# duckietown/gym-duckietown

Measured on NVIDIA H100. Metric: env-steps/sec (obs+reward+done) at N envs, 1/2/4/8 H100 vs CPU ref, higher is better.
Workload: dtype f64 logic / f32 raster / u8 obs

## Files before the change

gym-duckietown_b200/csrc/dts_maps.cu:

```cuda
#include <cstdarg>
#include <cstdio>
#include <cstring>
#include <type_traits>
#include <utility>
#include <vector>

#include "dts_kernels.h"

namespace dts {

struct MapSlot {
  DMap rec{};
  std::vector<void*> allocs;
  uint64_t hash = 0;
};

struct MapSlots {
  int n_envs;
  DMap* table = nullptr;
  std::vector<MapSlot> slots;
  std::vector<MapCounts> counts;
};

MapSlots* maps_create(const dts_config& cfg) {
  const size_t bytes = sizeof(DMap) * cfg.max_maps;
  void* t = nullptr;
  if (cudaMalloc(&t, bytes) != cudaSuccess) return nullptr;
  cudaMemset(t, 0, bytes);
  return new MapSlots{cfg.num_envs, static_cast<DMap*>(t), std::vector<MapSlot>(cfg.max_maps),
                      std::vector<MapCounts>(cfg.max_maps)};
}

void maps_destroy(MapSlots* m) {
  if (!m) return;
  for (const MapSlot& s : m->slots)
    for (void* p : s.allocs) cudaFree(p);
  cudaFree(m->table);
  delete m;
}

const DMap* maps_table(const MapSlots& m) { return m.table; }

const DMap* maps_get(const MapSlots& m, int slot) {
  return slot >= 0 && slot < (int)m.slots.size() && m.slots[slot].rec.valid ? &m.slots[slot].rec : nullptr;
}

const std::vector<MapCounts>& maps_counts(const MapSlots& m) { return m.counts; }

int maps_slot_count(const MapSlots& m) { return (int)m.slots.size(); }

uint64_t maps_hash(const MapSlots& m, int slot) { return maps_get(m, slot) ? m.slots[slot].hash : 0; }

namespace {
struct Hasher {
  uint64_t h = 0xcbf29ce484222325ull;
  void bytes(const void* p, size_t n) {
    const uint8_t* b = static_cast<const uint8_t*>(p);
    size_t i = 0;
    for (; i + 8 <= n; i += 8) {
      uint64_t w;
      memcpy(&w, b + i, 8);
      h = (h ^ w) * 0x100000001b3ull;
    }
    for (; i < n; i++) h = (h ^ b[i]) * 0x100000001b3ull;
  }
  template <typename T> void arr(const T* p, size_t count) {
    const uint64_t c = p ? count : 0;
    bytes(&c, sizeof c);
    if (p && count) bytes(p, count * sizeof(T));
  }
  template <typename T> void val(const T& v) { bytes(&v, sizeof v); }
  uint64_t done() const {
    uint64_t z = h;
    z = (z ^ (z >> 30)) * 0xbf58476d1ce4e5b9ull;
    z = (z ^ (z >> 27)) * 0x94d049bb133111ebull;
    z ^= z >> 31;
    return z ? z : 1;
  }
};
}

static uint64_t blob_hash(const dts_map_blob& b) {
  Hasher H;
  const size_t T = (size_t)b.grid_w * b.grid_h;
  H.val(b.tile_size); H.val(b.grid_w); H.val(b.grid_h);
  H.arr(b.tile_kind, T); H.arr(b.tile_angle, T); H.arr(b.tile_drivable, T); H.arr(b.tile_tex, T);
  H.arr(b.tile_curve_off, T); H.arr(b.tile_curve_cnt, T);
  H.arr(b.curves, (size_t)b.n_curves * 12);
  H.arr(b.coll_corners, (size_t)b.n_coll * 8); H.arr(b.coll_norms, (size_t)b.n_coll * 4);
  H.arr(b.coll_centers, (size_t)b.n_coll * 3); H.arr(b.coll_radii, (size_t)b.n_coll);
  H.val(b.n_objects);
  for (int o = 0; o < b.n_objects; o++) { dts_object s = b.objects[o]; s.reserved = 0; H.val(s); }
  H.val(b.n_meshes);
  for (int i = 0; i < b.n_meshes; i++) { dts_mesh s = b.meshes[i]; s.reserved = 0; H.val(s); }
  H.arr(b.tri_pos, (size_t)b.n_tris * 9); H.arr(b.tri_nrm, (size_t)b.n_tris * 9); H.arr(b.tri_uv, (size_t)b.n_tris * 6);
  H.arr(b.tri_col, (size_t)b.n_tris * 9); H.arr(b.tri_tex, (size_t)b.n_tris);
  H.val(b.n_textures);
  for (int t = 0; t < b.n_textures; t++) {
    const dts_texture& s = b.textures[t];
    H.val(s.width); H.val(s.height);
    H.arr(s.rgba, (size_t)s.width * s.height * 4);
  }
  H.arr(b.tex_segment, b.tex_segment ? (size_t)b.n_textures : 0);
  if (b.tex_class) {
    size_t texels = 0;
    for (int t = 0; t < b.n_textures; t++) texels += (size_t)b.textures[t].width * b.textures[t].height;
    H.arr(b.tex_class, texels);
  }
  H.val(b.start_tile[0]); H.val(b.start_tile[1]); H.val(b.has_start_pose);
  for (int k = 0; k < 3; k++) H.val(b.start_pose[k]);
  H.val(b.agent_mesh);
  H.val(b.n_dyn);
  for (int s = 0; s < b.n_dyn; s++) { dts_dyn_object q = b.dyn[s]; q.reserved = 0; H.val(q); }
  return H.done();
}

static std::string format(const char* fmt, ...) {
  char buf[512];
  va_list ap;
  va_start(ap, fmt);
  vsnprintf(buf, sizeof buf, fmt, ap);
  va_end(ap);
  return buf;
}

static size_t pool_bytes(const dts_texture& s) { return ((size_t)s.width * s.height * 4 + 255) & ~size_t(255); }

static std::string validate(const dts_map_blob* b, int slot, int n_slots) {
  if (!b || slot < 0 || slot >= n_slots) return format("bad map_id %d", slot);
  if (b->n_objects > DTS_MAX_OBJECTS) return format("map has %d objects, limit %d", b->n_objects, DTS_MAX_OBJECTS);
  if (b->grid_w <= 0 || b->grid_h <= 0 || !(b->tile_size > 0)) return "invalid tile grid";
  if (b->n_dyn < 0 || b->n_dyn > DTS_MAX_DYN) return format("map has %d dynamic obstacles, limit %d", b->n_dyn, DTS_MAX_DYN);
  for (int o = 0; o < b->n_objects; o++) {
    const dts_object& s = b->objects[o];
    if (s.mesh_id < 0 || s.mesh_id >= b->n_meshes) return format("object %d: bad mesh_id", o);
    if (s.alt_tex_to >= b->n_textures || s.alt_tex_from >= b->n_textures) return format("object %d: alt texture out of range", o);
    if (s.dyn_slot >= b->n_dyn) return format("object %d: dyn_slot %d out of range", o, s.dyn_slot);
  }
  for (int i = 0; i < b->n_meshes; i++) {
    const dts_mesh& me = b->meshes[i];
    if (me.tri_offset < 0 || me.tri_count < 0 || (int64_t)me.tri_offset + me.tri_count > b->n_tris)
      return format("mesh %d: triangles %d .. %d past n_tris %d", i, me.tri_offset, me.tri_offset + me.tri_count, b->n_tris);
  }
  size_t pool = 0;
  for (int t = 0; t < b->n_textures; t++) {
    const dts_texture& s = b->textures[t];
    if (s.width <= 0 || s.height <= 0 || (s.width & (s.width - 1)) || (s.height & (s.height - 1)))
      return format("texture %d: %dx%d is not a power of two", t, s.width, s.height);
    if (s.width > (1 << 15) || s.height > (1 << 15)) return format("texture %d: %dx%d too large", t, s.width, s.height);
    pool += pool_bytes(s);
  }
  if (pool >= (size_t(1) << 32)) return "textures exceed 4 GB";
  for (int s = 0; s < b->n_dyn; s++) {
    const dts_dyn_object& q = b->dyn[s];
    if (q.kind != DTS_DYN_DUCKIE && q.kind != DTS_DYN_DUCKIEBOT && q.kind != DTS_DYN_TRAFFICLIGHT) return format("dyn %d: bad kind %d", s, q.kind);
    if (q.object_index < 0 || q.object_index >= b->n_objects || b->objects[q.object_index].dyn_slot != s)
      return format("dyn %d: object_index %d does not point back to this slot", s, q.object_index);
  }
  return "";
}

static DObject mesh_object(const dts_map_blob& b, int mesh_id, float& top) {
  const dts_mesh& me = b.meshes[mesh_id];
  DObject d{};
  d.mesh_id = mesh_id; d.tri_offset = me.tri_offset; d.tri_count = me.tri_count;
  d.seg_tex = (me.seg_flat_tex >= 0 && me.seg_flat_tex < b.n_textures) ? me.seg_flat_tex : -1;
  float lo[3] = {1e30f, 1e30f, 1e30f}, hi[3] = {-1e30f, -1e30f, -1e30f};
  for (int t = 0; t < me.tri_count * 3; t++)
    for (int k = 0; k < 3; k++) {
      const float v = b.tri_pos[((size_t)me.tri_offset * 3 + t) * 3 + k];
      lo[k] = v < lo[k] ? v : lo[k];
      hi[k] = v > hi[k] ? v : hi[k];
    }
  top = hi[0] > hi[1] ? hi[0] : hi[1];
  top = top > hi[2] ? top : hi[2];
  float r2 = 0.f;
  for (int k = 0; k < 3; k++) { d.centre[k] = 0.5f * (lo[k] + hi[k]); const float h = 0.5f * (hi[k] - lo[k]); r2 += h * h; }
  d.bound_rad = sqrtf(r2);
  return d;
}

template <typename T>
static std::string upload(T*& dst, const std::remove_const_t<T>* src, size_t count, std::vector<void*>& owned) {
  const size_t bytes = (count ? count : 1) * sizeof(T);
  void* d = nullptr;
  cudaError_t e = cudaMalloc(&d, bytes + 16);
  if (e != cudaSuccess) return format("cudaMalloc(%zu B) failed: %s", bytes, cudaGetErrorString(e));
  owned.push_back(d);
  cudaMemset(d, 0, bytes + 16);
  if (count && src && (e = cudaMemcpy(d, src, count * sizeof(T), cudaMemcpyHostToDevice)) != cudaSuccess)
    return format("cudaMemcpy H2D failed: %s", cudaGetErrorString(e));
  dst = static_cast<T*>(d);
  return "";
}

std::string maps_upload(MapSlots& ms, int slot, const dts_map_blob* blob) {
  std::string err = validate(blob, slot, (int)ms.slots.size());
  if (!err.empty()) return err;
  const dts_map_blob& b = *blob;
  DMap m{};
  const size_t T = (size_t)b.grid_w * b.grid_h;
  m.tile_size = b.tile_size; m.grid_w = b.grid_w; m.grid_h = b.grid_h; m.n_tiles = (int)T;
  m.n_coll = b.n_coll;
  std::vector<int32_t> drv;
  for (int j = 0; j < b.grid_h; j++)
    for (int i = 0; i < b.grid_w; i++)
      if (b.tile_kind[j * b.grid_w + i] >= 0 && b.tile_drivable[j * b.grid_w + i]) { drv.push_back(i); drv.push_back(j); }
  m.start_i = b.start_tile[0]; m.start_j = b.start_tile[1];
  if (m.start_i < 0 || m.start_j < 0 || m.start_i >= b.grid_w || m.start_j >= b.grid_h) { m.start_i = -1; m.start_j = -1; }
  m.has_start_pose = b.has_start_pose != 0;
  for (int k = 0; k < 3; k++) m.start_pose[k] = b.start_pose[k];
  m.n_drivable = (int)drv.size() / 2;
  MapCounts counts{m.n_tiles, b.n_objects, 0};
  std::vector<DObject> objs(b.n_objects);
  for (int o = 0; o < b.n_objects; o++) {
    const dts_object& s = b.objects[o];
    float top;
    DObject& d = objs[o] = mesh_object(b, s.mesh_id, top);
    d.tri_base = (int32_t)counts.n_tris;
    for (int k = 0; k < 3; k++) { d.pos[k] = (float)s.pos[k]; d.dpos[k] = s.pos[k]; }
    d.dyn_slot = s.dyn_slot;
    d.alt_from = s.alt_tex_from; d.alt_to = s.alt_tex_to;
    d.scale = s.scale; d.y_rot_deg = s.y_rot_deg; d.optional = s.optional;
    d.spawn_rad = top * 0.5f * s.scale + 0.25f;
    counts.n_tris += d.tri_count;
  }
  m.n_objects = b.n_objects;
  m.n_tris = b.n_tris;
  if (b.agent_mesh >= 0 && b.agent_mesh < b.n_meshes) {
    float top;
    m.agent = mesh_object(b, b.agent_mesh, top);
    m.agent.scale = 1.0f; m.agent.dyn_slot = -1; m.agent.alt_from = m.agent.alt_to = -1;
  }
  m.agent.tri_base = (int32_t)counts.n_tris;
  counts.n_tris += m.agent.tri_count;
  std::vector<DTexture> tex(b.n_textures);
  std::vector<size_t> off(b.n_textures);
  size_t pool_size = 0;
  for (int t = 0; t < b.n_textures; t++) {
    off[t] = pool_size;
    pool_size += pool_bytes(b.textures[t]);
  }
  const size_t class_off = pool_size ? pool_size : 256;
  std::vector<uint8_t> pool(class_off + class_off / 4, 0);
  size_t class_src = 0;
  for (int t = 0; t < b.n_textures; t++) {
    const dts_texture& s = b.textures[t];
    memcpy(pool.data() + off[t], s.rgba, (size_t)s.width * s.height * 4);
    if (b.tex_class) memcpy(pool.data() + class_off + off[t] / 4, b.tex_class + class_src, (size_t)s.width * s.height);
    class_src += (size_t)s.width * s.height;
    int lw = 0, lh = 0;
    while ((1 << lw) < s.width) lw++;
    while ((1 << lh) < s.height) lh++;
    tex[t].w = s.width; tex[t].h = s.height;
    tex[t].info = (uint32_t)(off[t] >> 8) | ((uint32_t)lw << 24) | ((uint32_t)lh << 28);
    tex[t].pad = 0;
  }
  m.n_textures = b.n_textures;
  m.tex_class_off = (uint32_t)class_off;
  std::vector<int16_t> seg(b.n_textures > 0 ? b.n_textures : 1);
  for (int t = 0; t < b.n_textures; t++) {
    const int v = b.tex_segment ? b.tex_segment[t] : -1;
    seg[t] = (int16_t)((v >= 0 && v < b.n_textures) ? v : t);
  }
  m.n_dyn = b.n_dyn;
  const size_t N = ms.n_envs, D = b.n_dyn;
  std::vector<DDyn> par(D);
  std::vector<double> st((size_t)DTS_DYN_FIELDS * D * N);
  for (size_t s = 0; s < D; s++) {
    const dts_dyn_object& q = b.dyn[s];
    DDyn& p = par[s];
    p.kind = q.kind; p.object_index = q.object_index; p.pos_y = q.pos[1];
    for (int k = 0; k < 4; k++) p.norms[k] = q.norms[k / 2][k % 2];
    p.safety_radius = q.safety_radius; p.walk_distance = q.walk_distance; p.wiggle = q.wiggle; p.angle0 = q.angle;
    p.follow_dist = q.follow_dist; p.velocity = q.velocity; p.gain = q.gain; p.trim = q.trim; p.radius = q.radius;
    p.k = q.k; p.limit = q.limit; p.wheel_dist = q.wheel_dist; p.robot_width = q.robot_width; p.robot_length = q.robot_length;
    double f[DTS_DYN_FIELDS] = {};
    f[DTS_DYN_PX] = q.pos[0]; f[DTS_DYN_PZ] = q.pos[2]; f[DTS_DYN_ANGLE] = q.angle;
    f[DTS_DYN_YROT] = q.angle * (180.0 / 3.14159265358979323846);
    for (int k = 0; k < 4; k++) { f[DTS_DYN_CORNERS + 2 * k] = q.corners[k][0]; f[DTS_DYN_CORNERS + 2 * k + 1] = q.corners[k][1]; }
    f[DTS_DYN_START_X] = q.pos[0]; f[DTS_DYN_START_Z] = q.pos[2];
    f[DTS_DYN_WAIT] = q.wait_time; f[DTS_DYN_VEL] = q.vel; f[DTS_DYN_TIME] = 0.0; f[DTS_DYN_ACTIVE] = 0.0;
    p.freq = q.freq; p.tl_first = -1; p.pad = 0;
    if (q.kind == DTS_DYN_TRAFFICLIGHT) f[DTS_DYN_PATTERN] = q.pattern ? 1.0 : 0.0;
    for (int k = 0; k < DTS_DYN_FIELDS; k++)
      for (size_t e = 0; e < N; e++) st[((size_t)k * D + s) * N + e] = f[k];
  }
  int tl_first = -1, tl_last = -1;
  for (size_t s = 0; s < D; s++)
    if (par[s].kind == DTS_DYN_TRAFFICLIGHT) { if (tl_first < 0) tl_first = (int)s; tl_last = (int)s; }
  for (size_t s = 0; s < D; s++) par[s].tl_first = tl_first;
  if (tl_first >= 0)
    for (size_t e = 0; e < N; e++) st[((size_t)DTS_DYN_SHOWN * D + tl_first) * N + e] = b.dyn[tl_last].pattern ? 1.0 : 0.0;
  std::vector<double> init((size_t)DTS_DYN_FIELDS * D);
  for (int k = 0; k < DTS_DYN_FIELDS; k++)
    for (size_t s = 0; s < D; s++) init[(size_t)k * D + s] = N ? st[((size_t)k * D + s) * N] : 0.0;
  MapSlot fresh;
  auto put = [&](auto*& dst, const auto* src, size_t count) { if (err.empty()) err = upload(dst, src, count, fresh.allocs); };
  put(m.tile_kind, b.tile_kind, T);
  put(m.tile_angle, b.tile_angle, T);
  put(m.tile_drivable, b.tile_drivable, T);
  put(m.tile_tex, b.tile_tex, T);
  put(m.tile_curve_off, b.tile_curve_off, T);
  put(m.tile_curve_cnt, b.tile_curve_cnt, T);
  put(m.curves, b.curves, (size_t)b.n_curves * 12);
  put(m.coll_corners, b.coll_corners, (size_t)b.n_coll * 8);
  put(m.coll_norms, b.coll_norms, (size_t)b.n_coll * 4);
  put(m.coll_centers, b.coll_centers, (size_t)b.n_coll * 3);
  put(m.coll_radii, b.coll_radii, (size_t)b.n_coll);
  put(m.drivable_ij, drv.data(), drv.size());
  put(m.objects, objs.data(), objs.size());
  put(m.tri_pos, b.tri_pos, (size_t)b.n_tris * 9);
  put(m.tri_nrm, b.tri_nrm, (size_t)b.n_tris * 9);
  put(m.tri_uv, b.tri_uv, (size_t)b.n_tris * 6);
  put(m.tri_col, b.tri_col, (size_t)b.n_tris * 9);
  put(m.tri_tex, b.tri_tex, (size_t)b.n_tris);
  put(m.tex_pool, pool.data(), pool.size());
  for (int t = 0; t < b.n_textures && err.empty(); t++) tex[t].rgba = m.tex_pool + off[t];
  put(m.textures, tex.data(), tex.size());
  put(m.tex_segment, seg.data(), seg.size());
  put(m.dyn, par.data(), par.size());
  put(m.dyn_state, st.data(), st.size());
  put(m.dyn_init, init.data(), init.size());
  m.valid = 1;
  if (err.empty()) {
    cudaError_t e = cudaDeviceSynchronize();
    if (e == cudaSuccess) e = cudaMemcpy(ms.table + slot, &m, sizeof(DMap), cudaMemcpyHostToDevice);
    if (e != cudaSuccess) err = format("map table update failed: %s", cudaGetErrorString(e));
  }
  if (err.empty()) {
    fresh.rec = m;
    fresh.hash = blob_hash(b);
    std::swap(ms.slots[slot], fresh);
    ms.counts[slot] = counts;
  }
  for (void* p : fresh.allocs) cudaFree(p);
  return err;
}

}
```

gym-duckietown_b200/csrc/dts_render.cu:

```cuda
#include <algorithm>
#include <cstddef>
#include <cstdlib>
#include <iterator>
#include <type_traits>
#include <utility>
#include <vector>

#include "dts_camera.cuh"
#include "dts_kernels.h"

namespace dts {

struct RemapTab {
  const int32_t* src_xy;
  const short4* cbox;
  const short4* fbox;
  const int32_t* cell_start;
  const uint16_t* cell_bins;
  const int32_t* home_start;
  const int4* home_ent;
  int ext_x, ext_y;
  const uint16_t* table_of_env;
};
constexpr int kRemapNone = 0, kRemapTable = 1, kRemapPool = 2;
// ... 202 lines not shown
  const Vtx* vs[3] = {&a, &b, &c};
  int X[3], Y[3];
  float zw[3], q[3];
  const float Wf = (float)ec.W, Hf = (float)ec.H;
#pragma unroll
  for (int k = 0; k < 3; k++) {
    const float iw = 1.0f / vs[k]->cw;
    const float nx = vs[k]->cx * iw, ny = vs[k]->cy * iw, nz = vs[k]->cz * iw;
    const float sx = (nx * 0.5f + 0.5f) * Wf;
    const float sy = (0.5f - ny * 0.5f) * Hf;
    X[k] = (int)rintf(sx * 64.0f);
    Y[k] = (int)rintf(sy * 64.0f);
    zw[k] = nz * 0.5f + 0.5f;
    q[k] = iw;
  }
  const long long area2 = (long long)(X[1] - X[0]) * (Y[2] - Y[0]) - (long long)(X[2] - X[0]) * (Y[1] - Y[0]);
  if (area2 == 0) return false;
  const int i1 = area2 < 0 ? 2 : 1, i2 = area2 < 0 ? 1 : 2;
  const int x0 = X[0], y0 = Y[0], x1 = X[i1], y1 = Y[i1], x2 = X[i2], y2 = Y[i2];
  int minx = min(x0, min(x1, x2)), maxx = max(x0, max(x1, x2));
  int miny = min(y0, min(y1, y2)), maxy = max(y0, max(y1, y2));
  int qx[4] = {x0, x1, x2, 0}, qy[4] = {y0, y1, y2, 0};
  if (d) {
    const float iw = 1.0f / d->cw;
    const float sx = ((d->cx * iw) * 0.5f + 0.5f) * Wf, sy = (0.5f - (d->cy * iw) * 0.5f) * Hf;
    const int X3 = (int)rintf(sx * 64.0f), Y3 = (int)rintf(sy * 64.0f);
    if (area2 > 0) { qx[1] = X[1]; qy[1] = Y[1]; qx[2] = X[2]; qy[2] = Y[2]; qx[3] = X3; qy[3] = Y3; }
    else { qx[1] = X3; qy[1] = Y3; qx[2] = X[2]; qy[2] = Y[2]; qx[3] = X[1]; qy[3] = Y[1]; }
#pragma unroll
    for (int k = 0; k < 4; k++) {
      const int k1 = (k + 1) & 3, k2 = (k + 2) & 3;
      const long long cr = (long long)(qx[k1] - qx[k]) * (qy[k2] - qy[k1]) - (long long)(qx[k2] - qx[k1]) * (qy[k1] - qy[k]);
      if (cr <= 0) return false;
    }
    minx = min(minx, X3); maxx = max(maxx, X3); miny = min(miny, Y3); maxy = max(maxy, Y3);
  }
  const int px0 = max(minx >> 6, 0), px1 = min(maxx >> 6, ec.W - 1);
  const int py0 = max(miny >> 6, 0), py1 = min(maxy >> 6, ec.H - 1);
  if (px0 > px1 || py0 > py1) return true;
  if (!d && (maxx >> 6) - (minx >> 6) < 3 && (maxy >> 6) - (miny >> 6) < 3) {
    const int ex[3] = {x1 - x0, x2 - x1, x0 - x2}, ey[3] = {y1 - y0, y2 - y1, y0 - y2};
    const int ax[3] = {0, x1 - x0, x2 - x0}, ay[3] = {0, y1 - y0, y2 - y0};
    int e00[3];
#pragma unroll
    for (int k = 0; k < 3; k++) {
      const int bias = (ey[k] > 0 || (ey[k] == 0 && ex[k] < 0)) ? 0 : 1;
      e00[k] = ex[k] * (py0 * kSub - y0 - ay[k]) - ey[k] * (px0 * kSub - x0 - ax[k]) - bias;
    }
    bool any = false;
    for (int py = 0; py <= py1 - py0; py++)
      for (int px = 0; px <= px1 - px0; px++) {
#pragma unroll
        for (int s = 0; s < 4; s++) {
          const int sx = px * kSub + sample_x(s), sy = py * kSub + sample_y(s);
          const int e0 = e00[0] + ex[0] * sy - ey[0] * sx, e1 = e00[1] + ex[1] * sy - ey[1] * sx, e2 = e00[2] + ex[2] * sy - ey[2] * sx;
          any |= (e0 | e1 | e2) >= 0;
        }
      }
    if (!any) return true;
  }
  PrimRec r;
  r.X0 = x0; r.Y0 = y0; r.X1 = x1; r.Y1 = y1; r.X2 = x2; r.Y2 = y2; r.X3 = x0; r.Y3 = y0;
  const float dx1 = (float)(x1 - x0) * 0.015625f, dy1 = (float)(y1 - y0) * 0.015625f;
  const float dx2 = (float)(x2 - x0) * 0.015625f, dy2 = (float)(y2 - y0) * 0.015625f;
  const float areaf = dx1 * dy2 - dx2 * dy1;
  const float ia = 1.0f / areaf;
  const Vtx* p0 = vs[0]; const Vtx* p1 = vs[i1]; const Vtx* p2 = vs[i2];
  const float q0 = q[0], q1 = q[i1], q2 = q[i2];
  const float v0[7] = {zw[0], q0, p0->u * q0, p0->v * q0, p0->r * q0, p0->g * q0, p0->b * q0};
  const float v1[7] = {zw[i1], q1, p1->u * q1, p1->v * q1, p1->r * q1, p1->g * q1, p1->b * q1};
  const float v2[7] = {zw[i2], q2, p2->u * q2, p2->v * q2, p2->r * q2, p2->g * q2, p2->b * q2};
  float f0[7], fx[7], fy[7];
#pragma unroll
  for (int at = 0; at < 7; at++) {
    const float d1 = v1[at] - v0[at], d2 = v2[at] - v0[at];
    f0[at] = v0[at];
    fx[at] = (d1 * dy2 - d2 * dy1) * ia;
    fy[at] = (d2 * dx1 - d1 * dx2) * ia;
  }
  r.z0 = f0[0]; r.zx = fx[0]; r.zy = fy[0];
  r.q0 = f0[1]; r.qx = fx[1]; r.qy = fy[1];
  r.u0 = f0[2]; r.ux = fx[2]; r.uy = fy[2];
  r.v0 = f0[3]; r.vx = fx[3]; r.vy = fy[3];
  r.r0 = f0[4]; r.rx = fx[4]; r.ry = fy[4];
  r.g0 = f0[5]; r.gx = fx[5]; r.gy = fy[5];
  r.b0 = f0[6]; r.bx = fx[6]; r.by = fy[6];
  r.id = id;
  r.ltq = (lat + 1) | ((tex + 1) << 16);
  r.tex = tex >= 0 ? ec.textures[tex].info : 0u;
  if (d) {
    r.ltq |= 1 << 24;
    r.X1 = qx[1]; r.Y1 = qy[1]; r.X2 = qx[2]; r.Y2 = qy[2]; r.X3 = qx[3]; r.Y3 = qy[3];
  }
  const unsigned act = __activemask();
  const int lane = threadIdx.x & 31, leader = __ffs(act) - 1;
  int slot = 0;
  if (lane == leader) slot = atomicAdd(&ec.ctx->n_prims, __popc(act));
  slot = __shfl_sync(act, slot, leader) + __popc(act & ((1u << lane) - 1u));
  if (slot >= ec.max_prims) { ec.ctx->overflow = 1; return true; }
  const int4* src = reinterpret_cast<const int4*>(&r);
  int4* dst = reinterpret_cast<int4*>(ec.prims + slot);
#pragma unroll
  for (int k = 0; k < 8; k++) dst[k] = src[k];
  return true;
}

__device__ __forceinline__ Vtx clip_lerp(const Vtx& in, const Vtx& out, float din, float dout) {
  const float t = din / (din - dout);
  Vtx o;
  const float* a = reinterpret_cast<const float*>(&in);
  const float* b = reinterpret_cast<const float*>(&out);
  float* c = reinterpret_cast<float*>(&o);
#pragma unroll
  for (int k = 0; k < 9; k++) { const float d = b[k] - a[k]; c[k] = a[k] + t * d; }
  return o;
}

__device__ __forceinline__ void clip_and_emit_warp(const EmitCtx& ec, const Vtx& a, const Vtx& b, const Vtx& c, int id,
                                                   int tex, int lat, int lane) {
  for (int p2 = 0; p2 < 6; p2++) {
    const int cnt = !(plane_dist(a, p2) >= 0.0f) + !(plane_dist(b, p2) >= 0.0f) + !(plane_dist(c, p2) >= 0.0f);
    if (cnt == 3) return;
  }
  GeoWarp& g = *ec.gw;
  __syncwarp();
  if (lane == 0) { g.poly[0][0] = a; g.poly[0][1] = b; g.poly[0][2] = c; }
  __syncwarp();
  int n = 3, cur = 0;
  for (int pl = 0; pl < 6; pl++) {
    const Vtx* P = g.poly[cur];
    const float dk = lane < n ? plane_dist(P[lane], pl) : 0.0f;
    const bool in1 = dk >= 0.0f;
    const unsigned valid = (1u << n) - 1u;
    const unsigned out_mask = __ballot_sync(0xffffffffu, lane < n && !in1);
    if (!out_mask) continue;
    const int k2 = (lane + 1 == n) ? 0 : lane + 1;
    const float dn = __shfl_sync(0xffffffffu, dk, k2 & 31);
    const bool in2 = dn >= 0.0f;
    const bool cross = lane < n && (in1 != in2);
    const unsigned keep_mask = __ballot_sync(0xffffffffu, lane < n && in1) & valid;
    const unsigned cross_mask = __ballot_sync(0xffffffffu, cross) & valid;
    const unsigned below = (1u << lane) - 1u;
    int pos = __popc(keep_mask & below) + __popc(cross_mask & below);
    Vtx* T = g.poly[cur ^ 1];
    if (lane < n) {
      if (in1) T[pos++] = P[lane];
      if (in1 && !in2) T[pos] = clip_lerp(P[lane], P[k2], dk, dn);
      else if (!in1 && in2) T[pos] = clip_lerp(P[k2], P[lane], dn, dk);
    }
    n = __popc(keep_mask) + __popc(cross_mask);
    cur ^= 1;
    __syncwarp();
    if (n < 3) return;
  }
  const Vtx* P = g.poly[cur];
  if (lane + 2 < n) setup_and_emit(ec, P[0], P[lane + 1], P[lane + 2], id, tex, lat);
  __syncwarp();
}

__device__ __forceinline__ void process_triangle_uniform(const EmitCtx& ec, const Vtx& a, const Vtx& b, const Vtx& c,
                                                         int id, int tex, int lat, int lane) {
  const int cls = classify(a, b, c);
  if (cls == 2) return;
  if (cls == 0) { if (lane == 0) setup_and_emit(ec, a, b, c, id, tex, lat); }
  else clip_and_emit_warp(ec, a, b, c, id, tex, lat, lane);
}

__device__ __forceinline__ void process_triangle_lanes(const EmitCtx& ec, bool have, const Vtx& a, const Vtx& b,
                                                       const Vtx& c, int id, int tex, int lat, int lane) {
  const int cls = have ? classify(a, b, c) : 2;
  if (cls == 0) setup_and_emit(ec, a, b, c, id, tex, lat);
  unsigned need = __ballot_sync(0xffffffffu, cls == 1);
  while (need) {
    const int src = __ffs(need) - 1;
    need &= need - 1;
    Vtx va, vb, vc;
    const float* fa = reinterpret_cast<const float*>(&a);
    const float* fb = reinterpret_cast<const float*>(&b);
    const float* fc = reinterpret_cast<const float*>(&c);
#pragma unroll
    for (int k = 0; k < 9; k++) {
      reinterpret_cast<float*>(&va)[k] = __shfl_sync(0xffffffffu, fa[k], src);
      reinterpret_cast<float*>(&vb)[k] = __shfl_sync(0xffffffffu, fb[k], src);
      reinterpret_cast<float*>(&vc)[k] = __shfl_sync(0xffffffffu, fc[k], src);
    }
    const int sid = __shfl_sync(0xffffffffu, id, src), stex = __shfl_sync(0xffffffffu, tex, src);
    clip_and_emit_warp(ec, va, vb, vc, sid, stex, lat, lane);
  }
}

__device__ __forceinline__ bool box_overlaps(const int qx[4], const int qy[4], int n, int x_lo, int x_hi, int y_lo, int y_hi) {
#pragma unroll
  for (int k = 0; k < 4; k++) {
    if (k >= n) break;
    const int k1 = (k + 1) & 3;
    const int dx = qx[k1] - qx[k], dy = qy[k1] - qy[k];
    const int xs = (-dy > 0) ? x_hi : x_lo;
    const int ys = (dx > 0) ? y_hi : y_lo;
    const long long e = (long long)dx * (ys - qy[k]) - (long long)dy * (xs - qx[k]);
    if (e < 0) return false;
  }
  return true;
}
__device__ __forceinline__ bool bin_overlaps(const int qx[4], const int qy[4], int n, int ox, int oy) {
  return box_overlaps(qx, qy, n, ox + 8, ox + (kCoarseW - 1) * kSub + 56, oy + 8, oy + (kCoarseH - 1) * kSub + 56);
}

constexpr unsigned kRecGround = 0x100u;
constexpr unsigned kRecFlatOk = 0x200u;
__device__ __forceinline__ unsigned build_binrec(const PrimRec* __restrict__ pr, int p, int ox, int oy, BinRec* __restrict__ out,
                                                 const short4* __restrict__ fb = nullptr) {
  const int4 w0 = __ldg(reinterpret_cast<const int4*>(pr));
  const int4 w1 = __ldg(reinterpret_cast<const int4*>(pr) + 1);
  const float4 w2 = __ldg(reinterpret_cast<const float4*>(pr) + 2);
  const int ltq = __ldg(&pr->ltq);
  const int quad = (ltq >> 24) & 1;
  const int flat = (ltq & 0xffff) ? kKindFlat : 0;
  const int qx[4] = {w0.x, w0.z, w1.x, w1.z}, qy[4] = {w0.y, w0.w, w1.y, w1.w};
  const int nv = quad ? 4 : 3;
  unsigned live = 0xffu, inside = 0xffu;
  int E0[4] = {0, 0, 0, 0}, A[4] = {0, 0, 0, 0}, B[4] = {0, 0, 0, 0};
#pragma unroll
  for (int k = 0; k < 4; k++) {
    if (k >= nv) break;
    const int ka = k, kb = (k + 1) & 3;
    const int dx = qx[kb] - qx[ka], dy = qy[kb] - qy[ka];
    const int bias = (dy > 0 || (dy == 0 && dx < 0)) ? 0 : 1;
    long long e0 = (long long)dx * (oy - qy[ka]) - (long long)dy * (ox - qx[ka]) - bias;
    if (e0 < -(1LL << 30)) live = 0;
    if (e0 > (1LL << 30)) e0 = (1LL << 30);
    if (e0 < -(1LL << 30)) e0 = -(1LL << 30);
    const int a = -dy, b = dx, e = (int)e0;
    E0[k] = e; A[k] = a; B[k] = b;
    if (fb) {
    } else {
      const int hi = (a > 0 ? a * 504 : a * 8) + (b > 0 ? b * 248 : b * 8);
      const int lo = (a > 0 ? a * 8 : a * 504) + (b > 0 ? b * 8 : b * 248);
#pragma unroll
      for (int f = 0; f < 8; f++) {
        const int ef = e + a * ((f & 3) * kBinW * kSub) + b * ((f >> 2) * kBinH * kSub);
        if (ef + hi < 0) live &= ~(1u << f);
        if (ef + lo < 0) inside &= ~(1u << f);
      }
    }
  }
  if (fb) {
#pragma unroll 1
    for (int f = 0; f < 8; f++) {
      const short4 q = fb[f];
      if (q.z < q.x) { live &= ~(1u << f); continue; }
      const int X0 = q.x * kSub - ox + 8, X1 = q.z * kSub - ox + 56, Y0 = q.y * kSub - oy + 8, Y1 = q.w * kSub - oy + 56;
#pragma unroll
      for (int k = 0; k < 4; k++) {
        if (k >= nv) break;
        const int a = A[k], b = B[k], e = E0[k];
        const int hi = (a > 0 ? a * X1 : a * X0) + (b > 0 ? b * Y1 : b * Y0);
        const int lo = (a > 0 ? a * X0 : a * X1) + (b > 0 ? b * Y0 : b * Y1);
        if (e + hi < 0) live &= ~(1u << f);
        if (e + lo < 0) inside &= ~(1u << f);
      }
    }
  }
  int tiny = 0;
  if (!fb && !quad && live) {
    const int minx = min(qx[0], min(qx[1], qx[2])) - ox, maxx = max(qx[0], max(qx[1], qx[2])) - ox;
    const int miny = min(qy[0], min(qy[1], qy[2])) - oy, maxy = max(qy[0], max(qy[1], qy[2])) - oy;
    const int x0 = max(minx >> 6, 0), x1 = min(maxx >> 6, kCoarseW - 1), y0 = max(miny >> 6, 0), y1 = min(maxy >> 6, kCoarseH - 1);
    if (x1 - x0 < 4 && y1 - y0 < 4 && x1 >= x0 && y1 >= y0) {
      tiny = kKindTiny;
      E0[3] = x0 | (y0 << 16); A[3] = x1 | (y1 << 16);
    }
  }
  const int id = __float_as_int(w2.w);
  int4* o = reinterpret_cast<int4*>(out);
  o[0] = make_int4(E0[0], E0[1], E0[2], E0[3]);
  o[1] = make_int4(A[0], A[1], A[2], A[3]);
  o[2] = make_int4(B[0], B[1], B[2], B[3]);
  o[3] = make_int4(__float_as_int(w2.x), __float_as_int(w2.y), __float_as_int(w2.z), id);
  o[4] = make_int4(qx[0] - ox, qy[0] - oy, (int)((unsigned)p | (live << 16) | ((inside & live) << 24)),
                   (quad ? kKindQuad : 0) | (id < 2 ? kKindGround : 0) | tiny | flat);
  return (inside & live) | (id < 2 ? kRecGround : 0u) | ((flat || id < 2) && !tiny ? kRecFlatOk : 0u);
}

struct ShadeIn {
  const PrimRec* pr;
  int x0, y0;
  float q0, qx, qy, u0, ux, uy, v0, vx, vy, r0;
  int ltq;
  unsigned tex;
};
__device__ __forceinline__ ShadeIn load_shade(const PrimRec* __restrict__ prims, unsigned w) {
  const PrimRec* pr = prims + w;
  const int2 xy0 = __ldg(reinterpret_cast<const int2*>(pr));
  const float4 w3 = __ldg(reinterpret_cast<const float4*>(pr) + 3);
  const float4 w4 = __ldg(reinterpret_cast<const float4*>(pr) + 4);
  const float4 w5 = __ldg(reinterpret_cast<const float4*>(pr) + 5);
  ShadeIn si;
  si.pr = pr; si.x0 = xy0.x; si.y0 = xy0.y;
  si.q0 = w3.x; si.qx = w3.y; si.qy = w3.z; si.u0 = w3.w;
  si.ux = w4.x; si.uy = w4.y; si.v0 = w4.z; si.vx = w4.w;
  si.vy = w5.x; si.ltq = __float_as_int(w5.y); si.tex = __float_as_uint(w5.z); si.r0 = w5.w;
  return si;
}
__device__ __forceinline__ void shade_eval(const ShadeIn& si, const uint8_t* __restrict__ tex_pool, const float4* __restrict__ lat_tab,
                                           int pxa, int pya, float c3[3], float* qq_out = nullptr,
                                           const uint8_t* __restrict__ cls_pool = nullptr, int* cls_out = nullptr) {
  const float cdx = (float)(pxa + 32 - si.x0) * 0.015625f, cdy = (float)(pya + 32 - si.y0) * 0.015625f;
  float qq = fmaf(si.qy, cdy, fmaf(si.qx, cdx, si.q0));
  if (!(qq > 1e-20f)) qq = 1e-20f;
  if (qq_out) *qq_out = qq;
  const float rq = 1.0f / qq;
  const float u = fmaf(si.uy, cdy, fmaf(si.ux, cdx, si.u0)) * rq;
  const float v = fmaf(si.vy, cdy, fmaf(si.vx, cdx, si.v0)) * rq;
  const int ltq = si.ltq;
  const int lat = (ltq & 0xffff) - 1;
  if (lat >= 0) {
    const float fa_ = u * 7.0f, fb_ = (1.0f - v) * 7.0f;
    int ia = __float2int_rd(fa_), ib = __float2int_rd(fb_);
    ia = ia < 0 ? 0 : (ia > 6 ? 6 : ia);
    ib = ib < 0 ? 0 : (ib > 6 ? 6 : ib);
    const float fa = fa_ - (float)ia, fb = fb_ - (float)ib;
    const float4* L = lat_tab + lat * 64 + ia * 8 + ib;
    const bool lower = fb <= fa;
    const float4 c00 = L[0], c11 = L[9], cm = L[lower ? 8 : 1];
    const float t1 = lower ? fa : fb, t2 = lower ? fb : fa;
    c3[0] = fmaf(t2, c11.x - cm.x, fmaf(t1, cm.x - c00.x, c00.x));
    c3[1] = fmaf(t2, c11.y - cm.y, fmaf(t1, cm.y - c00.y, c00.y));
    c3[2] = fmaf(t2, c11.z - cm.z, fmaf(t1, cm.z - c00.z, c00.z));
  } else {
    const float4 w6 = __ldg(reinterpret_cast<const float4*>(si.pr) + 6);
    const float4 w7 = __ldg(reinterpret_cast<const float4*>(si.pr) + 7);
    c3[0] = fmaf(w6.y, cdy, fmaf(w6.x, cdx, si.r0)) * rq;
    c3[1] = fmaf(w7.x, cdy, fmaf(w6.w, cdx, w6.z)) * rq;
    c3[2] = fmaf(w7.w, cdy, fmaf(w7.z, cdx, w7.y)) * rq;
  }
  if (cls_out) *cls_out = 0;
  if (ltq & 0x00ff0000) {
    const unsigned ti = si.tex;
    const int lw = (ti >> 24) & 15, lh = ti >> 28;
    const int tw = 1 << lw, th = 1 << lh;
    const float twf = __int_as_float((127 + lw) << 23), thf = __int_as_float((127 + lh) << 23);
    const float tx = u * twf - 0.5f, ty = v * thf - 0.5f;
    const int txi = __float2int_rd(tx), tyi = __float2int_rd(ty);
    const float ffx = tx - (float)txi, ffy = ty - (float)tyi;
    const unsigned ti0 = (unsigned)txi & (tw - 1), ti1 = (ti0 + 1) & (tw - 1);
    const unsigned tj0 = (unsigned)tyi & (th - 1), tj1 = (tj0 + 1) & (th - 1);
    const unsigned r0 = tj0 << lw, r1 = tj1 << lw;
    const uchar4* tp = reinterpret_cast<const uchar4*>(tex_pool + ((size_t)(ti & 0xffffffu) << 8));
    const uchar4 t00 = __ldg(tp + (r0 + ti0)), t10 = __ldg(tp + (r0 + ti1));
    const uchar4 t01 = __ldg(tp + (r1 + ti0)), t11 = __ldg(tp + (r1 + ti1));
    const float a0[3] = {(float)t00.x, (float)t00.y, (float)t00.z}, a1[3] = {(float)t10.x, (float)t10.y, (float)t10.z};
    const float b0[3] = {(float)t01.x, (float)t01.y, (float)t01.z}, b1[3] = {(float)t11.x, (float)t11.y, (float)t11.z};
#pragma unroll
    for (int ch = 0; ch < 3; ch++) {
      const float ta = fmaf(ffx, a1[ch] - a0[ch], a0[ch]);
      const float tb = fmaf(ffx, b1[ch] - b0[ch], b0[ch]);
      const float tc = fmaf(ffy, tb - ta, ta);
      c3[ch] = tc * (c3[ch] * 0.00392156862745098f);
    }
    if (cls_out) {
      const unsigned cu = (unsigned)__float2int_rd(u * twf) & (tw - 1), cv = (unsigned)__float2int_rd(v * thf) & (th - 1);
      *cls_out = __ldg(cls_pool + ((size_t)(ti & 0xffffffu) << 6) + ((cv << lw) + cu));
    }
  }
}
__device__ __forceinline__ void shade_prim(const PrimRec* __restrict__ prims, unsigned w, const uint8_t* __restrict__ tex_pool,
                                           const float4* __restrict__ lat_tab, int pxa, int pya, float c3[3], float* qq_out = nullptr,
                                           const uint8_t* __restrict__ cls_pool = nullptr, int* cls_out = nullptr) {
  const ShadeIn si = load_shade(prims, w);
  shade_eval(si, tex_pool, lat_tab, pxa, pya, c3, qq_out, cls_pool, cls_out);
}

__device__ __forceinline__ uint32_t smem_u32(const void* p) { return (uint32_t)__cvta_generic_to_shared(p); }
__device__ __forceinline__ void mbar_init(uint64_t* bar, int count) {
  asm volatile("mbarrier.init.shared::cta.b64 [%0], %1;" ::"r"(smem_u32(bar)), "r"(count) : "memory");
}
__device__ __forceinline__ void mbar_fence_init() {
  asm volatile("fence.mbarrier_init.release.cluster;" ::: "memory");
  asm volatile("fence.proxy.async.shared::cta;" ::: "memory");
}
__device__ __forceinline__ void mbar_expect_tx(uint64_t* bar, uint32_t bytes) {
  asm volatile("mbarrier.arrive.expect_tx.shared::cta.b64 _, [%0], %1;" ::"r"(smem_u32(bar)), "r"(bytes) : "memory");
}
__device__ __forceinline__ void bulk_load(void* dst_smem, const void* src_gmem, uint32_t bytes, uint64_t* bar) {
  asm volatile("cp.async.bulk.shared::cluster.global.mbarrier::complete_tx::bytes [%0], [%1], %2, [%3];" ::"r"(smem_u32(dst_smem)),
               "l"(src_gmem), "r"(bytes), "r"(smem_u32(bar))
               : "memory");
}
__device__ __forceinline__ void mbar_wait(uint64_t* bar, uint32_t parity) {
  uint32_t ok;
  do {
    asm volatile("{\n .reg .pred p;\n mbarrier.try_wait.parity.shared::cta.b64 p, [%1], %2;\n selp.u32 %0, 1, 0, p;\n}"
                 : "=r"(ok)
                 : "r"(smem_u32(bar)), "r"(parity)
                 : "memory");
  } while (!ok);
}

__device__ __forceinline__ unsigned pack_rgb(float r, float g, float b) {
  const unsigned ur = min(__float2uint_rn(r * 255.0f), 255u);
  const unsigned ug = min(__float2uint_rn(g * 255.0f), 255u);
  const unsigned ub = min(__float2uint_rn(b * 255.0f), 255u);
  return ur | (ug << 8) | (ub << 16);
}

struct StoreLane {
  int src_lo, src_hi;
  int sh8;
  int off;
  int j, row;
};
__device__ __forceinline__ StoreLane make_store_lane(int lane, int W) {
  StoreLane sl;
  const int j = lane & 7, rowbase = lane & ~7;
  const int p0 = (4 * j) / 3;
  sl.sh8 = (4 * j - 3 * p0) * 8;
  sl.src_lo = rowbase + min(p0, 7);
  sl.src_hi = rowbase + min(p0 + 1, 7);
  sl.off = (lane >> 3) * W * 3 + 4 * j;
  sl.j = j; sl.row = lane >> 3;
  return sl;
}
__device__ __forceinline__ void store_bin_fast(uint8_t* __restrict__ bin0, const StoreLane& sl, unsigned rgb, int rows_ok) {
  const unsigned lo = __shfl_sync(0xffffffffu, rgb, sl.src_lo);
  const unsigned hi = __shfl_sync(0xffffffffu, rgb, sl.src_hi);
  const unsigned word = __funnelshift_r(lo | (hi << 24), hi >> 8, sl.sh8);
  if (sl.j < 6 && sl.row < rows_ok) *reinterpret_cast<unsigned*>(bin0 + sl.off) = word;
}
__device__ __forceinline__ void store_bin(uint8_t* __restrict__ out, unsigned rgb, int lane, int bx, int by, int W, int H) {
  const int gx = bx * kBinW + (lane & 7), gy = by * kBinH + (lane >> 3);
  if ((W & 3) == 0 && bx * kBinW + kBinW <= W) {
    const int j = lane & 7, rowbase = lane & ~7;
    const int p0 = (4 * j) / 3, sh8 = (4 * j - 3 * p0) * 8;
    const unsigned lo = __shfl_sync(0xffffffffu, rgb, rowbase + min(p0, 7));
    const unsigned hi = __shfl_sync(0xffffffffu, rgb, rowbase + min(p0 + 1, 7));
    const unsigned long long both = (unsigned long long)lo | ((unsigned long long)hi << 24);
    if (j < 6 && gy < H)
      *reinterpret_cast<unsigned*>(out + ((size_t)gy * W + bx * kBinW) * 3 + 4 * j) = (unsigned)(both >> sh8);
  } else if (gx < W && gy < H) {
    uint8_t* d = out + ((size_t)gy * W + gx) * 3;
    d[0] = (uint8_t)(rgb & 255); d[1] = (uint8_t)((rgb >> 8) & 255); d[2] = (uint8_t)(rgb >> 16);
  }
}

__device__ __forceinline__ void store_bin_planar_u8(uint8_t* __restrict__ out, int layout, unsigned rgb, int lane, int bx, int by,
                                                    int W, int H) {
  const int j = lane < 24 ? lane : 0, c = j >> 3;
  int s0, step;
  size_t addr;
  if (layout == DTS_OBS_CHW) {
    const int r = (j & 7) >> 1, h = j & 1;
    s0 = r * 8 + 4 * h; step = 1;
    addr = ((size_t)c * H + by * kBinH + r) * W + bx * kBinW + 4 * h;
  } else {
    const int xi = j & 7;
    s0 = xi; step = 8;
    addr = ((size_t)c * W + bx * kBinW + xi) * H + by * kBinH;
  }
  const unsigned p0 = __shfl_sync(0xffffffffu, rgb, s0), p1 = __shfl_sync(0xffffffffu, rgb, s0 + step);
  const unsigned p2 = __shfl_sync(0xffffffffu, rgb, s0 + 2 * step), p3 = __shfl_sync(0xffffffffu, rgb, s0 + 3 * step);
  const unsigned sel = (unsigned)c | ((unsigned)(4 + c) << 4);
  const unsigned word = __byte_perm(__byte_perm(p0, p1, sel), __byte_perm(p2, p3, sel), 0x5410);
  if (lane < 24) *reinterpret_cast<unsigned*>(out + addr) = word;
}

__device__ __forceinline__ void store_bin_any(uint8_t* __restrict__ out, int fmt, unsigned rgb, int lane, int bx, int by,
                                              int W, int H) {
  if (fmt == 0) { store_bin(out, rgb, lane, bx, by, W, H); return; }
  const int gx = bx * kBinW + (lane & 7), gy = by * kBinH + (lane >> 3);
  if (gx < W && gy < H) store_px_fmt(out, fmt & 3, fmt >> 2, gx, gy, W, H, rgb);
}

__host__ __device__ __forceinline__ bool lean_output(int layout, int dtype, int W) {
  return layout == DTS_OBS_HWC && dtype == DTS_OBS_U8 && (W & 3) == 0;
}

__device__ __forceinline__ unsigned fine_rows_in_image(int cby, int H) { return ((cby * kCFY + 1) * kBinH < H) ? 0xffu : 0x0fu; }
__device__ __forceinline__ unsigned fine_in_image(int cbx, unsigned rows, int W) {
  const int nx = min(kCFX, (W - cbx * kCoarseW + kBinW - 1) / kBinW);
  const unsigned cols = (1u << nx) - 1u;
  return rows & (cols | (cols << 4));
}

struct RemapPx { bool valid; int x, y; };
__device__ __forceinline__ RemapPx remap_source(const RemapTab& rt, int bx, int by, int lane, int W, int H) {
  const int gx = min(bx * kBinW + (lane & 7), W - 1), gy = min(by * kBinH + (lane >> 3), H - 1);
  const int sxy = __ldg(rt.src_xy + gy * W + gx);
  const int sx = (int)(short)(sxy & 0xffff), sy = sxy >> 16;
  return RemapPx{sx != -32768, sx * kSub, sy * kSub};
}
__device__ __forceinline__ RemapTab remap_of_env(RemapTab rt, int env, int W, int H, int cbins) {
  const int t = __ldg(rt.table_of_env + env);
  rt.src_xy += (size_t)t * W * H;
  rt.cbox += (size_t)t * cbins;
  rt.fbox += (size_t)t * cbins * (kCFX * kCFY);
  rt.cell_start += (size_t)t * (cbins + 1);
  rt.home_start += (size_t)t * (cbins + 1);
  return rt;
}

__device__ __forceinline__ void store_bin_lean(uint8_t* __restrict__ out, const StoreLane& sl, unsigned rgb, int lane, int bx, int by,
                                               int W, int H) {
  if (bx * kBinW + kBinW <= W) store_bin_fast(out + ((size_t)(by * kBinH) * W + bx * kBinW) * 3, sl, rgb, min(kBinH, H - by * kBinH));
  else store_bin(out, rgb, lane, bx, by, W, H);
}

__device__ __forceinline__ float depth_of(float qmax, bool px_valid = true) { return (px_valid && qmax > 0.0f) ? 1.0f / qmax : 0.0f; }
__device__ __forceinline__ void store_depth(float* __restrict__ dep, float d, int lane, int bx, int by, int W, int H) {
  const int gx = bx * kBinW + (lane & 7), gy = by * kBinH + (lane >> 3);
  if (gx < W && gy < H) dep[(size_t)gy * W + gx] = d;
}

struct LabelMap { const DObject* objects; int n_cells, n_objects, agent_base, tess; };
__device__ __forceinline__ LabelMap label_map(const DMap& m, int tess) {
  return LabelMap{m.objects, m.grid_w * m.grid_h, m.n_objects, m.agent.tri_base, tess};
}
__device__ __forceinline__ int tile_label(int tess, int id) {
  return id < 2 ? 1 : 2 + (tess ? (id - 2) / kTessTris : (id - 2) >> 1);
}
__device__ __forceinline__ int label_of_id(const LabelMap& lm, int id) {
  const int r = id - 2 - tile_draw_ids(lm.tess != 0) * lm.n_cells;
  if (r < 0) return tile_label(lm.tess, id);
  if (r >= lm.agent_base) return 2 + lm.n_cells + lm.n_objects;
  int lo = 0, hi = lm.n_objects - 1;
  while (lo < hi) {
    const int mid = (lo + hi + 1) >> 1;
    if (__ldg(&lm.objects[mid].tri_base) <= r) lo = mid; else hi = mid - 1;
  }
  return 2 + lm.n_cells + lo;
}
__device__ __forceinline__ void store_marking(uint8_t* __restrict__ mf, int v, int lane, int bx, int by, int W, int H) {
  const int gx = bx * kBinW + (lane & 7), gy = by * kBinH + (lane >> 3);
  if (gx < W && gy < H) mf[(size_t)gy * W + gx] = (uint8_t)v;
}
__device__ __forceinline__ void store_label(int16_t* __restrict__ lf, int v, int lane, int bx, int by, int W, int H) {
  const int gx = bx * kBinW + (lane & 7), gy = by * kBinH + (lane >> 3);
  if (gx < W && gy < H) lf[(size_t)gy * W + gx] = (int16_t)v;
}

constexpr int kAuxDepth = 1, kAuxLabels = 2, kAuxMarks = 4;
__host__ __device__ constexpr bool takes_winner(int aux) { return (aux & (kAuxLabels | kAuxMarks)) != 0; }
__host__ __device__ constexpr bool may_store_depth(int aux) { return (aux & (kAuxDepth | kAuxMarks)) != 0; }
__host__ __device__ constexpr bool needs_qq(int aux) { return takes_winner(aux) || may_store_depth(aux); }
template <int kAux>
__device__ __forceinline__ bool stores_depth(const float* depth) { return (kAux & kAuxDepth) || ((kAux & kAuxMarks) && depth); }

struct AuxFrames { AuxTargets t; size_t off; };
__device__ __forceinline__ AuxFrames aux_frames(const AuxTargets& aux, int env, int W, int H) {
  return AuxFrames{aux, (size_t)env * W * H};
}
template <int kAux>
__device__ __forceinline__ void store_aux(const AuxFrames& af, float depth, int label, int mark, int lane, int bx, int by, int W,
                                          int H) {
  if (stores_depth<kAux>(af.t.depth)) store_depth(af.t.depth + af.off, depth, lane, bx, by, W, H);
  if (kAux & kAuxLabels) store_label(af.t.labels + af.off, label, lane, bx, by, W, H);
  if (kAux & kAuxMarks) store_marking(af.t.marks + af.off, mark, lane, bx, by, W, H);
}

struct AuxPx { float qmax; int lab, mk; };
template <int kAux, typename LabelOf>
__device__ __forceinline__ void take_winner(AuxPx& pix, float qq, unsigned w, int c, const LabelOf& label_of) {
  if (!(qq >= pix.qmax)) return;
  const int l = label_of(w);
  if (qq > pix.qmax || l < pix.lab) {
    pix.qmax = qq; pix.lab = l;
    if constexpr ((kAux & kAuxMarks) != 0) pix.mk = c;
  } else if constexpr ((kAux & kAuxMarks) != 0) {
    if (l == pix.lab) pix.mk = min(pix.mk, c);
  }
}

__device__ __forceinline__ void clear_colour(const DState& S, const RenderCfg& rc, int env, float clr[3]) {
  const bool seg = (rc.mode & DTS_RENDER_SEGMENT) != 0;
  clr[0] = seg ? 1.0f : S.rep[env].horizon[0];
  clr[1] = seg ? 0.0f : S.rep[env].horizon[1];
  clr[2] = seg ? 1.0f : S.rep[env].horizon[2];
}

}

struct FrameMem {
  FrameCtx* ctx;
  PrimRec* prims;
  uint32_t* pairs;
  BinRec* recs;
  int* bin_count;
  int* bin_start;
  float4* lat;
  uint2* geo_list;
  uint2* solo;
  uint2* flat;
  int* work;
  int32_t* status;
};
constexpr int kWorkRaster = 0;
constexpr int kWorkPairPool = 1;
constexpr int kWorkGeoList = 2;
constexpr int kWorkSoloList = 3;
constexpr int kWorkFlatList = 4;

__host__ __device__ inline size_t align256(size_t b) { return (b + 255) & ~size_t(255); }

struct Renderer {
  int n, W, H, flags;
  int sms;
  int cbins;
  int max_prims = 0, max_lat = 0, items_max = 0, pool = 0;
  void* frame = nullptr;
  FrameMem fm{};
  RemapTab fish{};
  RemapTab rect{};
};

__host__ size_t carve(const Renderer& r, uintptr_t base, FrameMem& f) {
  const size_t n = r.n;
  size_t o = 0;
  auto take = [&](auto*& p, size_t count) {
    p = reinterpret_cast<std::remove_reference_t<decltype(p)>>(base + o);
    o += align256(count * sizeof(*p));
  };
  take(f.work, 64);
  take(f.ctx, n);
  take(f.bin_count, n * r.cbins);
  take(f.bin_start, n * r.cbins);
  take(f.prims, n * r.max_prims);
  take(f.pairs, r.pool);
  take(f.recs, r.pool);
  take(f.lat, n * r.max_lat * 64);
  take(f.geo_list, n * r.items_max);
  take(f.solo, n * r.cbins);
  take(f.flat, n * r.cbins);
  return o + 256;
}

__global__ void __launch_bounds__(128) k_frame_setup(const DState S, const DMap* __restrict__ maps, RenderCfg rc, FrameMem fm) {
  const int slot = blockIdx.x * blockDim.x + threadIdx.x;
  if (slot >= n_listed(rc.env_list, rc.env_count, rc.n_envs)) return;
  const int env = listed_env(rc.env_list, slot);
  FrameCtx& c = fm.ctx[env];
  const RenderEp ep = S.rep[env];
  double V[12];
  if (rc.mode & DTS_RENDER_TOP_DOWN) {
    const DMap& m = maps[S.map_id[env]];
    top_down_view((double)m.grid_w, (double)m.grid_h, m.tile_size, (double)ep.cam_fov_y_deg, V);
  } else {
    camera_view(S.pos_x[env], S.pos_z[env], S.angle[env], ep, (rc.flags & DTS_FLAG_DOMAIN_RAND) != 0, V);
  }
#pragma unroll
  for (int k = 0; k < 12; k++) c.V[k] = V[k];
  const double f = 1.0 / tan((double)ep.cam_fov_y_deg * kDeg2Rad / 2.0), aspect = (double)rc.width / (double)rc.height;
  const double zn = 0.04, zf = 100.0;
  c.P00 = (float)(f / aspect); c.P11 = (float)f;
  c.P22 = (float)((zf + zn) / (zn - zf)); c.P23 = (float)(2.0 * zf * zn / (zn - zf));
  c.n_prims = 0; c.n_lat = 0; c.overflow = 0; c.pad = 0;
}

__device__ __forceinline__ bool sphere_outside(float P00, float P11, float cx_, float cy_, float cz_, float rad) {
  const float hx = rsqrtf(P00 * P00 + 1.0f), hy = rsqrtf(P11 * P11 + 1.0f);
  bool out = cz_ - rad > -0.04f;
  out |= (P00 * cx_ + cz_) * hx > rad * 1.01f;
  out |= (-P00 * cx_ + cz_) * hx > rad * 1.01f;
  out |= (P11 * cy_ + cz_) * hy > rad * 1.01f;
  out |= (-P11 * cy_ + cz_) * hy > rad * 1.01f;
  return out;
}
// ... 1410 lines not shown
```

Baseline: 2.658 million.

## Store bilinear 2x2 texel footprints per texel for single 16-byte fetch

Each texel in the texture pool now holds its right, down and diagonal neighbours as a 16-byte record, so bilinear sampling makes one uint4 load instead of four scattered uchar4 loads. The class-pool offset scaling is adjusted to match the new pool layout. This cuts load instructions and address arithmetic per sample, but quadruples texture memory and its cache footprint, which can raise L1/L2 miss rates.

```diff
diff --git a/gym-duckietown_b200/csrc/dts_maps.cu b/gym-duckietown_b200/csrc/dts_maps.cu
--- a/gym-duckietown_b200/csrc/dts_maps.cu
+++ b/gym-duckietown_b200/csrc/dts_maps.cu
@@ -124,7 +124,23 @@
   return buf;
 }
 
-static size_t pool_bytes(const dts_texture& s) { return ((size_t)s.width * s.height * 4 + 255) & ~size_t(255); }
+static size_t pool_bytes(const dts_texture& s) { return ((size_t)s.width * s.height * 16 + 255) & ~size_t(255); }
+
+static void footprints(const dts_texture& s, uint8_t* dst) {
+  const uint8_t* t = s.rgba;
+  const size_t w = (size_t)s.width, h = (size_t)s.height;
+  for (size_t j = 0; j < h; j++) {
+    const size_t j1 = (j + 1) & (h - 1);
+    for (size_t i = 0; i < w; i++) {
+      const size_t i1 = (i + 1) & (w - 1);
+      uint8_t* e = dst + (j * w + i) * 16;
+      memcpy(e, t + (j * w + i) * 4, 4);
+      memcpy(e + 4, t + (j * w + i1) * 4, 4);
+      memcpy(e + 8, t + (j1 * w + i) * 4, 4);
+      memcpy(e + 12, t + (j1 * w + i1) * 4, 4);
+    }
+  }
+}
 
 static std::string validate(const dts_map_blob* b, int slot, int n_slots) {
   if (!b || slot < 0 || slot >= n_slots) return format("bad map_id %d", slot);
@@ -242,12 +258,12 @@
     pool_size += pool_bytes(b.textures[t]);
   }
   const size_t class_off = pool_size ? pool_size : 256;
-  std::vector<uint8_t> pool(class_off + class_off / 4, 0);
+  std::vector<uint8_t> pool(class_off + class_off / 16, 0);
   size_t class_src = 0;
   for (int t = 0; t < b.n_textures; t++) {
     const dts_texture& s = b.textures[t];
-    memcpy(pool.data() + off[t], s.rgba, (size_t)s.width * s.height * 4);
-    if (b.tex_class) memcpy(pool.data() + class_off + off[t] / 4, b.tex_class + class_src, (size_t)s.width * s.height);
+    footprints(s, pool.data() + off[t]);
+    if (b.tex_class) memcpy(pool.data() + class_off + off[t] / 16, b.tex_class + class_src, (size_t)s.width * s.height);
     class_src += (size_t)s.width * s.height;
     int lw = 0, lh = 0;
     while ((1 << lw) < s.width) lw++;
diff --git a/gym-duckietown_b200/csrc/dts_render.cu b/gym-duckietown_b200/csrc/dts_render.cu
--- a/gym-duckietown_b200/csrc/dts_render.cu
+++ b/gym-duckietown_b200/csrc/dts_render.cu
@@ -528,6 +528,7 @@
   si.vy = w5.x; si.ltq = __float_as_int(w5.y); si.tex = __float_as_uint(w5.z); si.r0 = w5.w;
   return si;
 }
+__device__ __forceinline__ float texel_ch(unsigned w, int ch) { return (float)((w >> (8 * ch)) & 0xffu); }
 __device__ __forceinline__ void shade_eval(const ShadeIn& si, const uint8_t* __restrict__ tex_pool, const float4* __restrict__ lat_tab,
                                            int pxa, int pya, float c3[3], float* qq_out = nullptr,
                                            const uint8_t* __restrict__ cls_pool = nullptr, int* cls_out = nullptr) {
@@ -569,14 +570,14 @@
     const float tx = u * twf - 0.5f, ty = v * thf - 0.5f;
     const int txi = __float2int_rd(tx), tyi = __float2int_rd(ty);
     const float ffx = tx - (float)txi, ffy = ty - (float)tyi;
-    const unsigned ti0 = (unsigned)txi & (tw - 1), ti1 = (ti0 + 1) & (tw - 1);
-    const unsigned tj0 = (unsigned)tyi & (th - 1), tj1 = (tj0 + 1) & (th - 1);
-    const unsigned r0 = tj0 << lw, r1 = tj1 << lw;
-    const uchar4* tp = reinterpret_cast<const uchar4*>(tex_pool + ((size_t)(ti & 0xffffffu) << 8));
-    const uchar4 t00 = __ldg(tp + (r0 + ti0)), t10 = __ldg(tp + (r0 + ti1));
-    const uchar4 t01 = __ldg(tp + (r1 + ti0)), t11 = __ldg(tp + (r1 + ti1));
-    const float a0[3] = {(float)t00.x, (float)t00.y, (float)t00.z}, a1[3] = {(float)t10.x, (float)t10.y, (float)t10.z};
-    const float b0[3] = {(float)t01.x, (float)t01.y, (float)t01.z}, b1[3] = {(float)t11.x, (float)t11.y, (float)t11.z};
+    const unsigned ti0 = (unsigned)txi & (tw - 1), tj0 = (unsigned)tyi & (th - 1);
+    const uint4* tp = reinterpret_cast<const uint4*>(tex_pool + ((size_t)(ti & 0xffffffu) << 8));
+    const uint4 fp = __ldg(tp + ((tj0 << lw) + ti0));
+    const unsigned t00 = fp.x, t10 = fp.y, t01 = fp.z, t11 = fp.w;
+    const float a0[3] = {texel_ch(t00, 0), texel_ch(t00, 1), texel_ch(t00, 2)};
+    const float a1[3] = {texel_ch(t10, 0), texel_ch(t10, 1), texel_ch(t10, 2)};
+    const float b0[3] = {texel_ch(t01, 0), texel_ch(t01, 1), texel_ch(t01, 2)};
+    const float b1[3] = {texel_ch(t11, 0), texel_ch(t11, 1), texel_ch(t11, 2)};
 #pragma unroll
     for (int ch = 0; ch < 3; ch++) {
       const float ta = fmaf(ffx, a1[ch] - a0[ch], a0[ch]);
@@ -586,7 +587,7 @@
     }
     if (cls_out) {
       const unsigned cu = (unsigned)__float2int_rd(u * twf) & (tw - 1), cv = (unsigned)__float2int_rd(v * thf) & (th - 1);
-      *cls_out = __ldg(cls_pool + ((size_t)(ti & 0xffffffu) << 6) + ((cv << lw) + cu));
+      *cls_out = __ldg(cls_pool + ((size_t)(ti & 0xffffffu) << 4) + ((cv << lw) + cu));
     }
   }
 }
```

After: 2.732 million, median of 6. +2.8%, better.
